# simon-donike/NIR-GAN

Measured on AMD Instinct MI355X. Metric: 256x256 RGB tiles/sec (G+D fwd+bwd+step), higher is better.
Workload: dtype f32 (3xbf16 split, 6 products, f32 accumulate) for the contractions with 32-channel runs incl. the Winograd plane GEMMs; exact f32 MFMA for the first / last layers; f32 everywhere else; 1 GPU; configs[1]: 6-block ResnetGenerator + 3-layer PatchGAN, bs=16/GPU, 256x256, GAN+L1, padding=0, fp32-equivalent MFMA (three bf16 terms, six products); global_batch=16, parallelism=dp1

## Files before the change

### include/nirgan_hip.h

```cpp
#ifndef NIRGAN_HIP_H
#define NIRGAN_HIP_H

#include <stdint.h>

#ifdef __cplusplus
extern "C" {
#endif

#define NIRGAN_MAX_TAPS 16

#define NIRGAN_OK 0
#define NIRGAN_ERR_ARG (-1)
#define NIRGAN_ERR_LAUNCH (-2)

#define NIRGAN_ACT_NONE 0
#define NIRGAN_ACT_RELU 1
#define NIRGAN_ACT_LRELU 2
#define NIRGAN_ACT_TANH 3

#define NIRGAN_BORDER_KEEP 0
#define NIRGAN_BORDER_REFLECT 1

int nirgan_version(void);
const char* nirgan_last_error(void);
// ... 142 lines not shown
    float* dbias;
} nirgan_tap_scatter_desc;
int nirgan_tap_scatter(const nirgan_tap_scatter_desc* d, void* stream);

typedef struct {
    const float* x; int x_hp, x_wp;
    int B, OH, OW, crop, C, k;
    const float* w;
    const float* bias; int act;
    float* out;
    const float* dout;
    float* dz; int64_t dz_elems;
    float* gx;
    float* gw; float* gbias;
    float* ws; int64_t ws_elems;
} nirgan_endconv_desc;
int64_t nirgan_endconv_dz_elems(int B, int OH, int OW);
int64_t nirgan_endconv_ws_elems(int B, int OH, int OW);
int nirgan_endconv_fwd(const nirgan_endconv_desc* d, void* stream);
int nirgan_endconv_dz(const nirgan_endconv_desc* d, void* stream);
int nirgan_endconv_dgrad(const nirgan_endconv_desc* d, void* stream);
int nirgan_endconv_wgrad(const nirgan_endconv_desc* d, void* stream);

int nirgan_lsgan(const float* pred, int64_t n, float target, float weight,
                 float* loss_out, float* grad, void* stream);

#define NIRGAN_GAN_VANILLA 1
#define NIRGAN_GAN_WGANGP 2
int nirgan_gan_loss(const float* pred, int64_t n, int mode, float target, float weight,
                    float* loss_out, float* grad, void* stream);

typedef struct {
    const float* rgb;
    const float* nir; const float* pred;
    int B, H, W;
    float w_l1, w_ndvi, w_ndwi, w_gndvi, w_savi, w_msavi, w_evi;
    int criterion;
    int log_all;
    const float* extra; int extra_cs, extra_c; float extra_scale;
    float* sums;
    float* grad_pred;
    float* ws; int64_t ws_elems;
} nirgan_pix_loss_desc;
#define NIRGAN_PIX_LOSS_WS_ELEMS 8192
int nirgan_pix_loss(const nirgan_pix_loss_desc* d, void* stream);

// ... 314 lines not shown
```

### nir-gan_amd/csrc/instnorm.hip

```cpp
#include "instnorm_dev.h"
#include <type_traits>

namespace {

__device__ __forceinline__ void rg_reduce2(f32x4& s1, f32x4& s2, f32x4* lds, int tid, int q4, int nrg) {
    lds[tid] = s1;
    lds[256 + tid] = s2;
    __syncthreads();
    if (tid < q4) {
        f32x4 a = lds[tid], b = lds[256 + tid];
        for (int r = 1; r < nrg; ++r) {
            a += lds[r * q4 + tid];
            b += lds[256 + r * q4 + tid];
        }
        s1 = a;
        s2 = b;
    }
    __syncthreads();
}

struct InFwd {
    const float* y; int y16; int HW, W, H, C;
    int norm; float eps;
    float* mean; float* rstd;
// ... 120 lines not shown
    int h = (start + rg) / p.W, w = (start + rg) - h * p.W;
    for (int pix = start + rg; pix < end; pix += nrg, w += nrg) {
        while (w >= p.W) { w -= p.W; ++h; }
        f32x4 v = (ldy4(yb, size_t(pix) * p.C + q * 4, p.y16) - mean) * rstd;
        v = act4(v, p.act, p.slope);
        if (rb) v += ld4(rb + size_t(h) * p.r_row + size_t(w) * p.C + q * 4);
        if (p.border == NIRGAN_BORDER_REFLECT && p.o_pad > 0) {
            int hs[3], wsx[3];
            const int nh = halo_images(h, p.H, p.o_pad, hs), nw = halo_images(w, p.W, p.o_pad, wsx);
            for (int i = 0; i < nh; ++i)
                for (int j = 0; j < nw; ++j) {
                    const size_t off = size_t(hs[i]) * p.o_row + size_t(wsx[j]) * p.C + q * 4;
                    if (ob) st4(ob + off, v);
                    st4_twin(ob16, off, v);
                }
        } else {
            const size_t off = size_t(h + p.o_pad) * p.o_row + size_t(w + p.o_pad) * p.C + q * 4;
            if (ob) st4(ob + off, v);
            st4_twin(ob16, off, v);
        }
    }
}

__global__ __launch_bounds__(256) void in_bwd_pass1_kernel(const InBwd p) {
    __shared__ f32x4 lds[512];
    const int tid = threadIdx.x, chunk = blockIdx.x, b = blockIdx.y;
    const int q4 = p.C / 4, nrg = in_nrg(p.C);
    const int q = tid % q4, rg = tid / q4;
    f32x4 s1 = {0, 0, 0, 0}, s2 = {0, 0, 0, 0};
    if (rg < nrg) {
        f32x4 mean = {0, 0, 0, 0}, rstd = {1, 1, 1, 1};
        if (p.norm) {
            mean = ld4(p.mean + size_t(b) * p.C + q * 4);
            rstd = ld4(p.rstd + size_t(b) * p.C + q * 4);
        }
        const float* gb = p.g ? y_at(p.g, size_t(b) * p.g_img, p.g16) : nullptr;
        const float* g2b = p.g2 ? p.g2 + size_t(b) * p.HW * p.C : nullptr;
        const float* yb = p.y ? y_at(p.y, size_t(b) * p.HW * p.C, p.y16) : nullptr;
        float* db = p.dy + size_t(b) * p.d_img + p.d_org;
        const int start = chunk * p.ppc;
        int end = start + p.ppc;
        end = end < p.HW ? end : p.HW;
        int h = (start + rg) / p.W, w = (start + rg) - h * p.W;
        for (int pix = start + rg; pix < end; pix += nrg, w += nrg) {
            while (w >= p.W) { w -= p.W; ++h; }
            const f32x4 ga = in_bwd_gsum(p, gb, g2b, h, w, pix, q);
            if (p.gsum_out) st4(p.gsum_out + (size_t(b) * p.HW + pix) * p.C + q * 4, ga);
            f32x4 z = {0, 0, 0, 0};
            const bool masked = p.act == NIRGAN_ACT_RELU || p.act == NIRGAN_ACT_LRELU;
            if (p.norm || masked) z = (ldy4(yb, size_t(pix) * p.C + q * 4, p.y16) - mean) * rstd;
            f32x4 gz = ga;
            if (masked) {
                const float neg = p.act == NIRGAN_ACT_RELU ? 0.f : p.slope;
#pragma unroll
                for (int i = 0; i < 4; ++i) gz[i] = z[i] > 0.f ? gz[i] : gz[i] * neg;
            }
            if (!p.norm) {
                const size_t off = size_t(h) * p.d_row + size_t(w) * p.C + q * 4;
                st4(db + off, gz);
                st4_twin(p.dy16 ? p.dy16 + size_t(b) * p.d_img + p.d_org : nullptr, off, gz);
            }
            s1 += gz;
            if (p.norm) s2 += gz * z;
        }
    }
    rg_reduce2(s1, s2, lds, tid, q4, nrg);
    if (tid < q4) {
        if (p.norm) {
            float* w = p.ws + (size_t(b) * p.nchunk + chunk) * 2 * p.C;
            st4(w + tid * 4, s1);
            st4(w + p.C + tid * 4, s2);
        } else if (p.dbias) {
            st4(p.ws + (size_t(b) * p.nchunk + chunk) * p.C + tid * 4, s1);
// ... 310 lines not shown
#define NG_APPLY_R(Y16, OUT, REFLECT) do { if (d->residual) NG_APPLY(Y16, OUT, REFLECT, true); else NG_APPLY(Y16, OUT, REFLECT, false); } while (0)
#define NG_APPLY_B(Y16, OUT) do { if (reflect) NG_APPLY_R(Y16, OUT, true); else NG_APPLY_R(Y16, OUT, false); } while (0)
#define NG_APPLY_O(Y16) do { if (out == 0) NG_APPLY_B(Y16, 0); else if (out == 1) NG_APPLY_B(Y16, 1); else NG_APPLY_B(Y16, 2); } while (0)
            if (p.y16) NG_APPLY_O(true); else NG_APPLY_O(false);
#undef NG_APPLY_O
#undef NG_APPLY_B
#undef NG_APPLY_R
#undef NG_APPLY
        } else {
            hipLaunchKernelGGL(in_apply_kernel, grid, dim3(256), 0, st, p);
        }
    }
    return nirgan_check_launch("instnorm_fwd");
}

extern "C" int nirgan_instnorm_bwd(const nirgan_in_bwd_desc* d, void* stream) {
    NG_REQUIRE(d && (d->dy || d->norm) && (d->g || d->g2), "instnorm_bwd: null pointer");
    const bool sums_only = d->dy == nullptr && d->dy_bf16 == nullptr;
    NG_REQUIRE(d->B > 0 && d->H > 0 && d->W > 0 && d->C >= 4 && d->C % 4 == 0 && d->C <= 1024, "instnorm_bwd: bad shape");
    NG_REQUIRE(!d->g || (d->g_hp == d->H + 2 * d->g_pad && d->g_wp == d->W + 2 * d->g_pad), "instnorm_bwd: g geometry mismatch");
    NG_REQUIRE(!d->g_fold || (d->g_pad < d->H && d->g_pad < d->W), "instnorm_bwd: fold halo wider than the image");
    NG_REQUIRE(sums_only || (d->d_hp == d->H + 2 * d->d_pad && d->d_wp == d->W + 2 * d->d_pad), "instnorm_bwd: dy geometry mismatch");
    const bool masked = d->act == NIRGAN_ACT_RELU || d->act == NIRGAN_ACT_LRELU;
    NG_REQUIRE(!(masked || d->norm) || d->y, "instnorm_bwd: y (pre-activation input of the block) required for the mask / statistics");
    NG_REQUIRE(!d->norm || (d->mean && d->rstd && d->ws), "instnorm_bwd: mean/rstd/ws required when norm");
    InBwd p = in_bwd_params(d);
    NG_REQUIRE(!d->dy_bf16 || (d->C % 8 == 0 && (reinterpret_cast<uintptr_t>(d->dy_bf16) & 15) == 0), "instnorm_bwd: bf16 twin needs C %% 8 == 0 and 16-byte alignment");
    NG_REQUIRE(!d->norm || d->ws_elems >= int64_t(d->B) * p.pchunks * 2 * d->C + int64_t(d->B) * 2 * d->C, "instnorm_bwd: ws too small");
    const bool pre = d->norm && d->sums_chunks > 0;
    NG_REQUIRE(!pre || d->gsum_out != nullptr || (d->g != nullptr && !d->g_fold && d->g2 == nullptr), "instnorm_bwd: sums_chunks needs the folded gradient in gsum_out, or a plain g (no fold, no g2)");
    hipStream_t st = static_cast<hipStream_t>(stream);
    NG_REQUIRE(d->norm || !d->dbias || (d->ws && d->ws_elems >= int64_t(d->B) * p.nchunk * d->C),
               "instnorm_bwd: dbias needs ws (one row of channel sums per block, summed in fixed order)");
    const long long gbig = (long long)p.g_img > (long long)p.d_img ? p.g_img : p.d_img;
    const bool fast = d->norm && d->g != nullptr && in_fast_ok(d->H, d->W, d->C, d->g_fold ? d->g_pad : 0, gbig > (long long)p.HW * p.C ? gbig : (long long)p.HW * p.C);
    const dim3 bgrid(p.nchunk, d->B);
#define NG_P1(Y16, G16, FOLD) hipLaunchKernelGGL((in_bwd_pass1_fast_kernel<Y16, G16, FOLD>), bgrid, dim3(256), 0, st, p)
#define NG_P1_F(Y16, G16) do { if (d->g_fold) NG_P1(Y16, G16, true); else NG_P1(Y16, G16, false); } while (0)
#define NG_P1_G(Y16) do { if (p.g16) NG_P1_F(Y16, true); else NG_P1_F(Y16, false); } while (0)
    if (!pre) {
        if (fast) { if (p.y16) NG_P1_G(true); else NG_P1_G(false); }
        else hipLaunchKernelGGL(in_bwd_pass1_kernel, bgrid, dim3(256), 0, st, p);
    }
#undef NG_P1_G
#undef NG_P1_F
#undef NG_P1
    if (!d->norm && d->dbias) return nirgan_colsum(d->ws, int64_t(d->B) * p.nchunk, d->C, d->dbias, 1, stream);
    if (d->norm) {
        hipLaunchKernelGGL(in_bwd_finalize_kernel, dim3(d->B, (d->C >= 64 && d->C % 64 == 0) ? d->C / 64 : 1), dim3(256), 0, st, p, d->B);
        if (!sums_only) {
            const bool fast2 = (d->g != nullptr ? fast : (d->gsum_out != nullptr && in_fast_ok(d->H, d->W, d->C, 0, (long long)p.d_img > (long long)p.HW * p.C ? p.d_img : (long long)p.HW * p.C)));
            const int dyo = d->dy && d->dy_bf16 ? 1 : (d->dy ? 0 : 2);
            const int B_ = d->B;
#define NG_P2(Y16, G16, FOLD, DY) hipLaunchKernelGGL((in_bwd_pass2_fast_kernel<Y16, G16, FOLD, DY>), bgrid, dim3(256), 0, st, p, B_)
#define NG_P2_D(Y16, G16, FOLD) do { if (dyo == 0) NG_P2(Y16, G16, FOLD, 0); else if (dyo == 1) NG_P2(Y16, G16, FOLD, 1); else NG_P2(Y16, G16, FOLD, 2); } while (0)
#define NG_P2_F(Y16, G16) do { if (d->g_fold && d->g) NG_P2_D(Y16, G16, true); else NG_P2_D(Y16, G16, false); } while (0)
#define NG_P2_G(Y16) do { if (p.g16) NG_P2_F(Y16, true); else NG_P2_F(Y16, false); } while (0)
            if (fast2) { if (p.y16) NG_P2_G(true); else NG_P2_G(false); }
            else hipLaunchKernelGGL(in_bwd_pass2_kernel, bgrid, dim3(256), 0, st, p, d->B);
#undef NG_P2_G
#undef NG_P2_F
#undef NG_P2_D
#undef NG_P2
        }
    }
// ... 3 lines not shown
```

### nir-gan_amd/nirgan_hip/engine.py

```python
from __future__ import annotations

import ctypes as C
from typing import Dict, List, Optional

import numpy as np
import torch

from . import geometry as G
from . import lib as L
from .options import OPT

IN_EPS = 1e-5


def _ptr(t: Optional[torch.Tensor]) -> Optional[int]:
    return None if t is None else t.data_ptr()


PRECISIONS = {"fp32": 0, "bf16": 1, "bf16x3": 2}


def precision_code(precision) -> int:
    if precision in PRECISIONS.values():
        return int(precision)
# ... 733 lines not shown
            continue
        for w in h.writers:
            if isinstance(w, L.InFwdDesc):
                w.out = None
            else:
                w.dy = None
            n += 1
        h.fp32_dead = True
    return n


def emit_in_bwd(plan: Plan, ctx: Ctx, *, g: Optional[Halo], g_fold=False, g2: Optional[Halo] = None, a: Optional[Halo] = None,
                act=L.ACT_NONE, slope=0.2, y: Optional[Halo] = None, stats=None, norm=True, dy: Halo, gsum: Optional[Halo] = None,
                dbias: Optional[torch.Tensor] = None, ws=None, shape=None, sums_only: bool = False, pre_sums: int = 0):
    B, H, W, Cc = shape
    d = L.InBwdDesc()
    if g is not None:
        assert g.H == H and g.W == W and g.C == Cc
        d.g, d.g_hp, d.g_wp, d.g_pad, d.g_fold = g.ptr_any(), g.hp, g.wp, g.pad, (1 if g_fold else 0)
        d.g_bf16 = 1 if g.is16 else 0
    if g2 is not None:
        assert g2.pad == 0
        d.g2 = g2.ptr
    d.act, d.slope = act, slope
    d.norm = 1 if norm else 0
    if y is not None:
        d.y, d.y_bf16 = y.ptr_any(), (1 if y.is16 else 0)
    if norm:
        d.mean, d.rstd = stats[0].data_ptr(), stats[1].data_ptr()
    if norm or dbias is not None:
        d.ws, d.ws_elems = ws.data_ptr(), ws.numel()
    d.B, d.H, d.W, d.C = B, H, W, Cc
    assert not sums_only or norm
    d.dy, d.d_hp, d.d_wp, d.d_pad = (None if sums_only else dy.operand_ptr()), dy.hp, dy.wp, dy.pad
    if dy.t16 is not None and not sums_only:
        d.dy_bf16 = dy.t16.data_ptr()
        dy.writers.append(d)
    if gsum is not None:
        d.gsum_out = gsum.ptr
    if pre_sums:
        assert norm and (gsum is not None or (g is not None and not g_fold and g2 is None))
        d.sums_chunks = pre_sums
    if dbias is not None:
        d.dbias = dbias.data_ptr()
    ctx.keep.append(d)
    plan.add("nirgan_instnorm_bwd", C.byref(d))
# ... 35 lines not shown
        self.inp, self.weight, self.bias = inp, weight, bias
        self.k, self.s, self.p, self.cout = k, s, p, cout
        self.norm, self.act, self.residual = norm, act, residual
        self.cin = inp.C if kind != "rowpacked" else cin_real
        ctx = eng.ctx
        if kind == "convT":
            self.OH, self.OW = inp.H * 2, inp.W * 2
        else:
            self.OH, self.OW = G.conv_out(inp.H, k, s, p), G.conv_out(inp.W, k, s, p)
        assert inp.pad >= (p if kind != "convT" else 1), (name, inp.pad, p)
        B = inp.B
        phase_px = self.OH * self.OW // (4 if kind == "convT" else 1)
        y16 = (ctx.precision == 1 and norm and OPT.bf16_y and OPT.epilogue_stats and cout % 4 == 0 and phase_px % 128 == 0
               and self.OH * self.OW >= min(OPT.epilogue_min_pixels, OPT.epilogue_min_pixels_bf16) and one_pass_tiles(B * phase_px, cout))
        self.y = Halo(ctx, B, self.OH, self.OW, cout, 0, bf16=y16)
        self.out = Halo(ctx, B, self.OH, self.OW, cout, out_pad, twin=True)
        eng.twinned.append(self.out)
        self.out_border = out_border
        self.stats = (ctx.zeros(B, cout), ctx.zeros(B, cout)) if norm else None
        eng.scratch.want(B, self.OH, self.OW, cout)
        self.keep_z = keep_z
        self.producer, self.defer_apply = None, False
        self.wino6, self.wino_fwd, self.wino_fwd_keeps_V = False, None, False

    def fold_producer_apply(self, producer: "ConvIN"):
        producer.defer_apply, self.producer = True, producer

    def emit_fwd(self, plan: Plan, pack: Plan):
        eng, ctx, inp = self.eng, self.eng.ctx, self.inp
        if self.kind == "conv" and wino_applicable(ctx, inp, self.k, self.s, self.p, self.cout, self.OH, self.OW):
            pre = self._emit_fwd_wino6(plan, pack)
        elif self.kind in ("conv", "rowpacked"):
            pre = self._emit_fwd_direct(plan, pack)
        else:
            descs = self._phase_descs(pack, inp, self.y, G.convT_fwd_phases(inp.H, inp.W, self.k, self.p),
                                      lambda hw: G.convT_fwd_pack(inp.C, self.cout, self.k, hw), self.bias, run=inp.C, N=self.cout,
                                      in_off=inp.pad - 1, out_off=0)
            pre = self._conv_stats(descs)
            emit_conv_group(plan, ctx, descs)
        emit_in_fwd(plan, ctx, self.y, self.out, norm=self.norm, act=(L.ACT_NONE if self.keep_z else self.act),
                    residual=self.residual, border=self.out_border, stats=self.stats, ws=(pre[2] if pre is not None else eng.scratch.get()),
                    stats_only=self.defer_apply, pre_stats=(pre[:2] if pre is not None else None))

    def _emit_fwd_wino6(self, plan: Plan, pack: Plan):
        eng, ctx, inp, k = self.eng, self.eng.ctx, self.inp, self.k
        keep = bool(eng.keep_wino_V)
        prod = self.producer
        xn = (prod.y, prod.stats, prod.act) if prod is not None and prod.defer_apply else None
        self.wino6 = True
        pre = sws = None
        if self.norm and OPT.epilogue_stats:
            T = _w6_tiles(inp.B, self.OH, self.OW, wino6_variant(k))
# ... 43 lines not shown
        return descs

    def _conv_stats(self, descs):
        pre = attach_conv_stats(self.eng.ctx, descs, self.bias) if self.norm else None
        self._y_fallback(pre, descs)
        return pre

    def _y_fallback(self, pre, descs):
        if self.y.is16 and pre is None:
            self.y = Halo(self.eng.ctx, self.inp.B, self.OH, self.OW, self.cout, 0)
            for d in descs:
                d.out, d.out_bf16 = self.y.ptr, 0

    def alloc_bwd(self, need_dgrad: bool):
        ctx, k = self.eng.ctx, self.k
        if self.kind == "convT":
            zpad = 1
        elif self.s == 1:
            zpad = k - 1 if need_dgrad else 0
        else:
            zpad = 1 if need_dgrad else 0
        self.dy = Halo(ctx, self.inp.B, self.OH, self.OW, self.cout, zpad, twin=True)
        self.eng.twinned.append(self.dy)

    def emit_bwd(self, plan: Plan, pack: Plan, *, g: Optional[Halo], g_fold=False, g2: Optional[Halo] = None,
                 gsum: Optional[Halo] = None, gw: Optional[torch.Tensor], gb: Optional[torch.Tensor], dgrad_out: Optional[Halo],
                 mask: Optional[Halo] = None, act=None):
        eng, ctx, inp = self.eng, self.eng.ctx, self.inp
        k, s, p = self.k, self.s, self.p
        act = self.act if act is None else act
        dy = self.dy
        w6_bwd = (self.kind == "conv" and s == 1 and gw is not None and dgrad_out is not None and dgrad_out.pad == p and dy.pad == k - 1
                  and wino_dgrad_applicable(ctx, k, s, dgrad_out, self.cout, inp.C) and inp.C > 64
                  and inp.pad == 1 and p == 1 and self.cout % 128 == 0)
        fuse_dy = (w6_bwd and k == 3 and self.norm and dy.t16 is None and OPT.fuse_dy_norm and wino6_variant(3) == 6
                   and act in (L.ACT_NONE, L.ACT_RELU, L.ACT_LRELU))
        scratch = eng.scratch.get()
        pre_sums, ws, gsum = (self._first_pass_from_w6_output(g, g_fold, g2, gsum, act)
                              or self._first_pass_from_conv_epilogues(g, g_fold, g2, gsum, act) or (0, scratch, gsum))
        nd = emit_in_bwd(plan, ctx, g=g, g_fold=g_fold, g2=g2, act=act, y=self.y, stats=self.stats, norm=self.norm, dy=self.dy, gsum=gsum,
                         dbias=(None if self.norm else gb),
                         ws=ws, shape=(inp.B, self.OH, self.OW, self.cout), pre_sums=pre_sums, sums_only=fuse_dy)
        if w6_bwd:
            self._emit_w6_backward(plan, pack, gw, dgrad_out, nd if fuse_dy else None)
        elif self.kind == "conv" and s == 1 and gw is not None and dgrad_out is not None:
            self._emit_paired_s1(plan, pack, gw, dgrad_out)
        else:
            if gw is not None:
                self._emit_wgrad(plan, gw)
            if dgrad_out is not None:
                self._emit_dgrad(plan, pack, dgrad_out, frozen=gw is None)

    def _first_pass_from_w6_output(self, g, g_fold, g2, gsum, act):
        ctx, inp = self.eng.ctx, self.inp
        od = g.w6_out_desc if g is not None else None
        if not (od is not None and od.r == 6 and g_fold and self.norm and g.pad == 1 and self.dy.t16 is None and OPT.fuse_inbwd):
            return None
        mo, Hp, Wp = _w6_geo(od.r if od.r else 3)[0], od.H, od.W
        if not (Hp == self.OH + 2 and Wp == self.OW + 2 and od.K == self.cout and od.B == inp.B and min(Hp, Wp) >= 6
                and (Hp - 3) // mo == (Hp - 1) // mo and (Wp - 3) // mo == (Wp - 1) // mo):
            return None
        chunks = (-(-Hp // mo)) * (-(-Wp // mo))
        if gsum is None:
# ... 179 lines not shown
```

### nir-gan_amd/nirgan_hip/lib.py

```python
from __future__ import annotations

import ctypes as C
import os

_HERE = os.path.dirname(os.path.abspath(__file__))
LIB_PATH = os.path.join(os.path.dirname(_HERE), "lib", "libnirgan_hip.so")

MAX_TAPS = 16
ACT_NONE, ACT_RELU, ACT_LRELU, ACT_TANH = 0, 1, 2, 3
BORDER_KEEP, BORDER_REFLECT = 0, 1
OP_CONV, OP_WGRAD, OP_IN_FWD, OP_IN_BWD = 1, 2, 3, 4

fp = C.c_void_p
i32, i64, f32 = C.c_int, C.c_int64, C.c_float


class ConvDesc(C.Structure):
    _fields_ = [("inp", fp), ("in_elems", i64), ("in_hp", i32), ("in_wp", i32), ("in_cs", i32),
                ("run", i32), ("in_stride", i32), ("in_oh", i32), ("in_ow", i32), ("ntaps", i32),
                ("tap_dh", i32 * MAX_TAPS), ("tap_dw", i32 * MAX_TAPS),
                ("w", fp), ("w_elems", i64), ("bias", fp),
                ("out", fp), ("out_elems", i64), ("out_hp", i32), ("out_wp", i32), ("out_cs", i32),
                ("out_stride", i32), ("out_oh", i32), ("out_ow", i32),
                ("B", i32), ("OH", i32), ("OW", i32), ("N", i32), ("zero_page", fp),
# ... 184 lines not shown

class RasterLookupDesc(C.Structure):
    _fields_ = [("points", fp), ("n_points", i32), ("H", i32), ("W", i32), ("dtype", i32), ("raster", fp),
                ("x0", C.c_double), ("dx", C.c_double), ("y0", C.c_double), ("dy", C.c_double),
                ("has_nodata", i32), ("nodata", i32), ("value", fp)]


class WinoDyDesc(C.Structure):
    _fields_ = [("dy", fp), ("dy_hp", i32), ("dy_wp", i32), ("dy_pad", i32), ("B", i32), ("H", i32), ("W", i32), ("K", i32),
                ("Yt", fp), ("Yt_elems", i64), ("r", i32)]


class Wino6Desc(C.Structure):
    _fields_ = [("x", fp), ("x_hp", i32), ("x_wp", i32), ("B", i32), ("H", i32), ("W", i32), ("C", i32), ("K", i32),
                ("U", fp), ("bias", fp), ("V", fp), ("V_elems", i64), ("M", fp), ("M_elems", i64), ("y", fp), ("zero_page", fp), ("r", i32), ("stats_ws", fp), ("stats_ws_elems", i64),
                ("fuse_y", fp), ("fuse_mean", fp), ("fuse_rstd", fp), ("fuse_g2", fp), ("fuse_gz", fp), ("fuse_part", fp), ("fuse_part_elems", i64),
                ("fuse_act", i32), ("fuse_slope", f32), ("algo", i32), ("U3", fp)]


W6_ONE_TILE, W6_DIRECT_TILE, W6_X3_R4 = 1, 3, 5
W6_PATCH_PER_THREAD, W6_PATCH_PER_LANES = 16, 17
WGRAD_ONE_UNIT, WGRAD_TILE128 = 1, 2
CONV_TILE128, CONV_X3_R4 = 1, 4


class EndConvDesc(C.Structure):
    _fields_ = [("x", fp), ("x_hp", i32), ("x_wp", i32), ("B", i32), ("OH", i32), ("OW", i32), ("crop", i32), ("C", i32), ("k", i32),
                ("w", fp), ("bias", fp), ("act", i32), ("out", fp), ("dout", fp), ("dz", fp), ("dz_elems", i64), ("gx", fp),
                ("gw", fp), ("gbias", fp), ("ws", fp), ("ws_elems", i64)]


class PlanEntry(C.Structure):
    _fields_ = [("op", i32), ("desc", fp)]


PROTOTYPES = {
    "nirgan_version": (i32, []),
    "nirgan_last_error": (C.c_char_p, []),
    "nirgan_conv_igemm": (i32, [C.POINTER(ConvDesc), fp]),
    "nirgan_wgrad_igemm": (i32, [C.POINTER(WgradDesc), fp]),
    "nirgan_conv_igemm_group": (i32, [C.POINTER(C.POINTER(ConvDesc)), i32, fp]),
    "nirgan_conv_wgrad_pair": (i32, [C.POINTER(ConvDesc), C.POINTER(WgradDesc), fp]),
    "nirgan_conv_kernel_name": (C.c_char_p, [C.POINTER(ConvDesc)]),
    "nirgan_wgrad_kernel_name": (C.c_char_p, [C.POINTER(WgradDesc)]),
    "nirgan_conv_wgrad_pair_kernel_name": (C.c_char_p, [C.POINTER(ConvDesc), C.POINTER(WgradDesc)]),
    "nirgan_reduce_rows": (i32, [fp, i32, i32, i32, fp, fp, i64, i32, i32, fp]),
# ... 44 lines not shown
    "nirgan_tile_metrics": (i32, [C.POINTER(TileMetricsDesc), fp]),
    "nirgan_window_stats": (i32, [C.POINTER(WindowStatsDesc), fp]),
    "nirgan_val_panel_ws_bytes": (i64, [i32, i32, i32]),
    "nirgan_val_panel": (i32, [C.POINTER(ValPanelDesc), fp]),
    "nirgan_class_metrics_ws_elems": (i64, [i32, i32, i32, i32]),
    "nirgan_class_metrics": (i32, [C.POINTER(ClassMetricsDesc), fp]),
    "nirgan_ssim_loss_ws_elems": (i64, [i32, i32, i32, i32]),
    "nirgan_ssim_loss": (i32, [C.POINTER(SsimLossDesc), fp]),
    "nirgan_emd_loss_ws_bytes": (i64, [i32, i64, i32]),
    "nirgan_emd_loss": (i32, [C.POINTER(EmdLossDesc), fp]),
    "nirgan_instnorm_ws_elems": (i64, [i32, i32, i32, i32]),
    "nirgan_instnorm_fwd": (i32, [C.POINTER(InFwdDesc), fp]),
    "nirgan_instnorm_bwd": (i32, [C.POINTER(InBwdDesc), fp]),
    "nirgan_nchw_to_halo": (i32, [fp, i32, i32, i32, i32, fp, i32, i32, i32, i32, i32, fp]),
    "nirgan_conv_channel_dgrad": (i32, [C.POINTER(ChanDgradDesc), fp]),
    "nirgan_tap_gather": (i32, [C.POINTER(TapGatherDesc), fp]),
    "nirgan_tap_scatter": (i32, [C.POINTER(TapScatterDesc), fp]),
    "nirgan_endconv_dz_elems": (i64, [i32, i32, i32]),
    "nirgan_endconv_ws_elems": (i64, [i32, i32, i32]),
    "nirgan_endconv_fwd": (i32, [C.POINTER(EndConvDesc), fp]),
    "nirgan_endconv_dz": (i32, [C.POINTER(EndConvDesc), fp]),
    "nirgan_endconv_dgrad": (i32, [C.POINTER(EndConvDesc), fp]),
    "nirgan_endconv_wgrad": (i32, [C.POINTER(EndConvDesc), fp]),
    "nirgan_lsgan": (i32, [fp, i64, f32, f32, fp, fp, fp]),
    "nirgan_gan_loss": (i32, [fp, i64, i32, f32, f32, fp, fp, fp]),
    "nirgan_pix_loss": (i32, [C.POINTER(PixLossDesc), fp]),
    "nirgan_pixmlp_fwd": (i32, [C.POINTER(PixMlpDesc), fp]),
    "nirgan_pixmlp_train": (i32, [C.POINTER(PixMlpDesc), fp]),
    "nirgan_pixmlp_ws_elems": (i64, [i32, i32, i32, i32]),
    "nirgan_pixdisc_ws_elems": (i64, [i32, i32, i32, i32]),
    "nirgan_pixdisc_fwd": (i32, [C.POINTER(PixDiscDesc), fp]),
    "nirgan_pixdisc_bwd": (i32, [C.POINTER(PixDiscDesc), fp]),
    "nirgan_adam": (i32, [fp, fp, fp, fp, i64, f32, f32, f32, f32, i32, fp]),
    "nirgan_bilinear_fwd": (i32, [fp, i32, i32, i32, fp, i32, i32, fp]),
    "nirgan_bilinear_bwd": (i32, [fp, i32, i32, i32, fp, i32, i32, fp]),
    "nirgan_inject_fwd": (i32, [C.POINTER(InjectFwdDesc), fp]),
    "nirgan_inject_bwd": (i32, [C.POINTER(InjectBwdDesc), fp]),
    "nirgan_param_scale_fwd": (i32, [fp, fp, fp, i64, fp]),
    "nirgan_param_scale_bwd": (i32, [fp, fp, fp, fp, fp, fp, i64, i64, fp]),
    "nirgan_colsum": (i32, [fp, i64, i32, fp, i32, fp]),
    "nirgan_fill": (i32, [fp, i64, f32, fp]),
    "nirgan_axpy": (i32, [fp, fp, i64, f32, fp]),
    "nirgan_run_plan": (i32, [C.POINTER(PlanEntry), i32, fp]),
}


# ... 52 lines not shown
```

### nir-gan_amd/nirgan_hip/nets.py

```python
from __future__ import annotations

import ctypes as C
from typing import Dict, Optional

import torch

from . import geometry as G
from . import lib as L
from .options import OPT
from .engine import (ConvIN, Ctx, Halo, LayerHost, Plan, TapPlaneConv, drop_dead_fp32_stores, emit_conv, grad_halo,
                     emit_deferred_reduce_rows, emit_w6_deferred_finishes, emit_wgrad, wino_applicable)


def generator_layout(n_blocks: int) -> dict:
    up0 = 10 + n_blocks
    return {"first": 1, "down": [4, 7], "blocks": list(range(10, 10 + n_blocks)), "up": [up0, up0 + 3], "last": up0 + 7}


class _Engine(LayerHost):
    def __init__(self, device, precision="fp32", keep_wino_V: bool = False):
        super().__init__(Ctx(device, precision), keep_wino_V)
        self.pack_fwd, self.pack_bwd = Plan(self.ctx), Plan(self.ctx)
        self.fwd, self.bwd = Plan(self.ctx), Plan(self.ctx)
        self._packed_version = -1
# ... 312 lines not shown
        self.bwd_pred = Plan(ctx)
        for plan, mode in ((b, "train"), (self.bwd_frozen, "input"), (self.bwd_pred, "pred")):
            frozen = mode != "train"

            def GW(i, what="weight"):
                return None if frozen else gr[f"model.{i}.{what}"]
            if not frozen:
                for k in ("model.0.bias", "model.11.bias"):
                    plan.add("nirgan_fill", gr[k].data_ptr(), gr[k].numel(), 0.0)
                ctx.rr_deferred = [] if OPT.batch_reduce else None
            self.C5.emit_bwd(plan, pk, GW(11), GW(11, "bias"))
            self.C4.emit_bwd(plan, pk, g=self.C5.gin, g_fold=False, gw=GW(8), gb=GW(8, "bias"), dgrad_out=self.g3p)
            if not frozen:
                emit_deferred_reduce_rows(plan, ctx, last=False)
                self.bwd_tail = (len(plan.ops), "model.8.weight", "model.11.bias")
            self.C3.emit_bwd(plan, pk, g=self.g3p, g_fold=False, gw=GW(5), gb=GW(5, "bias"), dgrad_out=self.g2)
            self.C2.emit_bwd(plan, pk, g=self.g2, gw=GW(2), gb=GW(2, "bias"), dgrad_out=self.g1)
            if not frozen:
                emit_deferred_reduce_rows(plan, ctx, last=False)
                self.bwd_mid = (len(plan.ops), "model.0.weight", "model.0.bias")
            self.C1.emit_bwd(plan, pk, g=self.g1, gw=GW(0), gb=GW(0, "bias"), dgrad_out=self.gx4 if mode == "input" else None)
            if not frozen:
                emit_deferred_reduce_rows(plan, ctx)
            if mode == "pred":
                d = L.ChanDgradDesc()
                dy, w = self.C1.dy, self.params["model.0.weight"]
                d.dy, d.dy_hp, d.dy_wp, d.dy_pad, d.C = dy.ptr, dy.hp, dy.wp, dy.pad, dy.C
                d.w, d.cin, d.k, d.stride, d.pad, d.channel = w.data_ptr(), 4, 4, 2, 1, 3
                d.B, d.H, d.W, d.out = B, self.H, self.W, self.gpred.data_ptr()
                ctx.keep.append(d)
                plan.add("nirgan_conv_channel_dgrad", C.byref(d))


class PixelDiscriminatorEngine(_DiscriminatorFrontEnd):

    FLAT_ELEMS = 8772

    def __init__(self, params: Dict[str, torch.Tensor], grads: Optional[Dict[str, torch.Tensor]], B: int, H: int, W: int,
                 need_backward: bool = True, precision="fp32"):
        w1 = params["net.0.weight"]
        super().__init__(params, grads, B, H, W, w1.device, precision)
        ctx = self.ctx
        ndf, in_nc = w1.shape[0], w1.shape[1]
        if in_nc != 4 or ndf != 64:
            raise NotImplementedError("the pixel discriminator of the MI355X path is built for cat(rgb, nir) = 4 channels and ndf = 64")
        if H * W < 2:
            raise ValueError(f"Expected more than 1 spatial element when training, got input size {torch.Size([B, 2 * ndf, H, W])}")
# ... 33 lines not shown
```

### nir-gan_amd/nirgan_hip/options.py

```python
from __future__ import annotations

import os


class Options:
    w6_gemm_algo: int = 0
    wgrad_algo: int = 0
    w6_pair: bool = True
    winograd: str = "f6"
    epilogue_stats: bool = True
    fuse_inbwd: bool = True
    epilogue_min_pixels: int = 16384
    epilogue_min_pixels_bf16: int = 1024
    fuse_dy_norm: bool = True
    dp_buckets: bool = True
    bf16_y: bool = True
    bf16_g: bool = True
    bf16_store_min_tiles: int = 100
    bf16_twin_only: bool = True
    fold_apply: bool = True
    tile256: bool = True
    batch_reduce: bool = True
    wgrad_target: int = 512
    split3: bool = True
    split3_wino: bool = True
    pair_phases: bool = True
    pair_pixels: bool = True
    x3_r4: bool = True
    endconv_direct: bool = True

    def reset(self):
        for k, v in vars(Options).items():
            if not k.startswith("_") and not callable(v):
                setattr(self, k, v)


    def update_from(self, text: str):
        for item in filter(None, (t.strip() for t in text.split(","))):
            k, _, v = item.partition("=")
            if not hasattr(Options, k) or k.startswith("_"):
                raise ValueError(f"NIRGAN_OPTIONS: unknown option '{k}'")
            cur = getattr(Options, k)
            setattr(self, k, (v.lower() in ("1", "true", "yes", "on")) if isinstance(cur, bool) else type(cur)(v))


OPT = Options()
if os.environ.get("NIRGAN_OPTIONS"):
    OPT.update_from(os.environ["NIRGAN_OPTIONS"])
```

Before: 1100 tiles/s.

## Add direct MFMA kernels for the discriminator's first 4->64 stride-2 conv

Adds a dedicated forward kernel for the PatchGAN's first Conv2d(4,64,4,s2,p1)+LeakyReLU. It gathers input patches straight from the padded input and runs exact f32 MFMA with a fused bias and activation epilogue, replacing the generic rowpacked conv path. It also adds direct wgrad and pred-dgrad kernels that take the LeakyReLU mask from the stored activation rather than the pre-activation, plus an instance-norm backward variant that does the same. The backward path sits behind an option that is off by default, so only the fused forward runs with default settings. Because the pre-activation is not stored, the mask is taken from the activation, which requires a positive slope.

```diff
diff --git a/include/nirgan_hip.h b/include/nirgan_hip.h
--- a/include/nirgan_hip.h
+++ b/include/nirgan_hip.h
@@ -188,6 +188,23 @@
 int nirgan_endconv_dgrad(const nirgan_endconv_desc* d, void* stream);
 int nirgan_endconv_wgrad(const nirgan_endconv_desc* d, void* stream);
 
+typedef struct {
+    const float* x;
+    int B, H, W, cin, cout, k;
+    const float* w;
+    const float* bias;
+    float slope;
+    float* a;
+    const float* g;
+    float* gw; float* gb;
+    float* ws; int64_t ws_elems;
+    float* gpred;
+} nirgan_firstconv_desc;
+int64_t nirgan_firstconv_ws_elems(int B, int H, int W);
+int nirgan_firstconv_fwd(const nirgan_firstconv_desc* d, void* stream);
+int nirgan_firstconv_wgrad(const nirgan_firstconv_desc* d, void* stream);
+int nirgan_firstconv_pred_dgrad(const nirgan_firstconv_desc* d, void* stream);
+
 int nirgan_lsgan(const float* pred, int64_t n, float target, float weight,
                  float* loss_out, float* grad, void* stream);
 
diff --git a/nir-gan_amd/csrc/firstconv.hip b/nir-gan_amd/csrc/firstconv.hip
--- /dev/null
+++ b/nir-gan_amd/csrc/firstconv.hip
@@ -0,0 +1,316 @@
+#include "common.h"
+
+namespace {
+
+constexpr int FC = 64;
+constexpr int FWD_MAX_BLOCKS = 512;
+constexpr int WG_MAX_BLOCKS = 512;
+constexpr int WG_ROW = FC * FC + FC;
+constexpr int PT_R = 14, PT_C = 30;
+
+struct FcP {
+    const float* x; int x_wp; int64_t x_img;
+    float* a; int a_wp; int64_t a_img;
+    const float* w; const float* bias; float slope;
+    int B, H, W, OH, OW;
+    const float* g;
+    float* ws; float* gw; float* gb; float* gpred;
+};
+
+__device__ __forceinline__ int uni(int v) { return __builtin_amdgcn_readfirstlane(v); }
+
+__global__ __launch_bounds__(256) void firstconv_fwd_kernel(const FcP p, const float* __restrict__ x, const float* __restrict__ w, float* __restrict__ a) {
+    const int lane = threadIdx.x & 63, half = lane >> 5, col = lane & 31;
+    float wa[32][2];
+#pragma unroll
+    for (int s = 0; s < 32; ++s) {
+        const int k = (s & 3) * 16 + (s >> 3) * 4 + 2 * ((s >> 2) & 1) + half;
+        wa[s][0] = w[col * FC + k];
+        wa[s][1] = w[(col + 32) * FC + k];
+    }
+    f32x4 bv[2][4];
+#pragma unroll
+    for (int t = 0; t < 2; ++t)
+#pragma unroll
+        for (int q = 0; q < 4; ++q) {
+            const f32x4 z = {0.f, 0.f, 0.f, 0.f};
+            bv[t][q] = p.bias ? *reinterpret_cast<const f32x4*>(p.bias + 32 * t + 8 * q + 4 * half) : z;
+        }
+    const int plane = p.OH * p.OW, npix = p.B * plane;
+    const int ntiles = (npix + 31) / 32, nwaves = uni(gridDim.x * 4);
+    const float slope = p.slope;
+
+    auto gather = [&](int tile, f32x4 (&xv)[4][2], int64_t& ooff) {
+        tile = tile < ntiles ? tile : ntiles - 1;
+        int pix = tile * 32 + col;
+        const bool ok = pix < npix;
+        pix = ok ? pix : npix - 1;
+        const int b = pix / plane, rem = pix - b * plane, oh = rem / p.OW, ow = rem - oh * p.OW;
+        const float* xp = x + (int64_t(b) * p.x_img + (int64_t(2 * oh) * p.x_wp + 2 * ow + half) * 4);
+#pragma unroll
+        for (int r = 0; r < 4; ++r)
+#pragma unroll
+            for (int j = 0; j < 2; ++j) xv[r][j] = *reinterpret_cast<const f32x4*>(xp + (r * p.x_wp + 2 * j) * 4);
+        ooff = ok ? int64_t(b) * p.a_img + (int64_t(oh + 1) * p.a_wp + ow + 1) * FC : -1;
+    };
+    auto tile_out = [&](const f32x4 (&xv)[4][2], int64_t ooff) {
+        f32x16 acc0 = {0}, acc1 = {0};
+#pragma unroll
+        for (int s = 0; s < 32; ++s) {
+            const float b = xv[s >> 3][(s >> 2) & 1][s & 3];
+            acc0 = __builtin_amdgcn_mfma_f32_32x32x2f32(wa[s][0], b, acc0, 0, 0, 0);
+            acc1 = __builtin_amdgcn_mfma_f32_32x32x2f32(wa[s][1], b, acc1, 0, 0, 0);
+        }
+        if (ooff < 0) return;
+        float* o = a + ooff + 4 * half;
+#pragma unroll
+        for (int q = 0; q < 4; ++q) {
+            f32x4 v0, v1;
+#pragma unroll
+            for (int i = 0; i < 4; ++i) {
+                const float z0 = acc0[4 * q + i] + bv[0][q][i], z1 = acc1[4 * q + i] + bv[1][q][i];
+                v0[i] = z0 > 0.f ? z0 : z0 * slope;
+                v1[i] = z1 > 0.f ? z1 : z1 * slope;
+            }
+            *reinterpret_cast<f32x4*>(o + 8 * q) = v0;
+            *reinterpret_cast<f32x4*>(o + 32 + 8 * q) = v1;
+        }
+    };
+    int tile = uni(blockIdx.x * 4 + (threadIdx.x >> 6));
+    f32x4 x0[4][2], x1[4][2];
+    int64_t o0, o1;
+    gather(tile, x0, o0);
+    while (true) {
+        if (tile >= ntiles) break;
+        gather(tile + nwaves, x1, o1);
+        asm volatile("" ::: "memory");
+        tile_out(x0, o0);
+        tile += nwaves;
+        if (tile >= ntiles) break;
+        gather(tile + nwaves, x0, o0);
+        asm volatile("" ::: "memory");
+        tile_out(x1, o1);
+        tile += nwaves;
+    }
+}
+
+__global__ __launch_bounds__(256) void firstconv_wgrad_kernel(const FcP p, const float* __restrict__ g, const float* __restrict__ a,
+                                                              const float* __restrict__ x, float* __restrict__ ws) {
+    __shared__ float red[WG_ROW];
+    const int lane = threadIdx.x & 63, wv = threadIdx.x >> 6, half = lane >> 5, col = lane & 31;
+    const int upr = (p.OW + 15) / 16, nunits = p.B * p.OH * upr, nwaves = uni(gridDim.x * 4);
+    const int xlane = ((col >> 3) * p.x_wp + ((col >> 1) & 3)) * 4 + 2 * (col & 1);
+    const float slope = p.slope;
+    struct Buf { f32x2 g[8], a[8], x[8]; };
+    auto load = [&](int unit, Buf& f) {
+        unit = unit < nunits ? unit : nunits - 1;
+        const int row = unit / upr, ow0 = (unit - row * upr) * 16;
+        const int b = row / p.OH, oh = row - b * p.OH;
+        const float* gu = g + int64_t(row) * p.OW * FC + 2 * col;
+        const float* au = a + (int64_t(b) * p.a_img + (int64_t(oh + 1) * p.a_wp + 1) * FC) + 2 * col;
+        const float* xu = x + (int64_t(b) * p.x_img + int64_t(2 * oh) * p.x_wp * 4) + xlane;
+#pragma unroll
+        for (int j = 0; j < 8; ++j) {
+            int ow = ow0 + 2 * j + half;
+            ow = ow < p.OW ? ow : p.OW - 1;
+            f.g[j] = *reinterpret_cast<const f32x2*>(gu + ow * FC);
+            f.a[j] = *reinterpret_cast<const f32x2*>(au + ow * FC);
+            f.x[j] = *reinterpret_cast<const f32x2*>(xu + ow * 8);
+        }
+    };
+    f32x16 acc[2][2] = {{{0}, {0}}, {{0}, {0}}};
+    float sb0 = 0.f, sb1 = 0.f;
+    auto mma = [&](int unit, const Buf& f) {
+        const int ow0 = (unit % upr) * 16;
+#pragma unroll
+        for (int j = 0; j < 8; ++j) {
+            const bool ok = ow0 + 2 * j + half < p.OW;
+            const float d0 = ok ? f.g[j][0] * (f.a[j][0] > 0.f ? 1.f : slope) : 0.f;
+            const float d1 = ok ? f.g[j][1] * (f.a[j][1] > 0.f ? 1.f : slope) : 0.f;
+            sb0 += d0;
+            sb1 += d1;
+            acc[0][0] = __builtin_amdgcn_mfma_f32_32x32x2f32(d0, f.x[j][0], acc[0][0], 0, 0, 0);
+            acc[0][1] = __builtin_amdgcn_mfma_f32_32x32x2f32(d0, f.x[j][1], acc[0][1], 0, 0, 0);
+            acc[1][0] = __builtin_amdgcn_mfma_f32_32x32x2f32(d1, f.x[j][0], acc[1][0], 0, 0, 0);
+            acc[1][1] = __builtin_amdgcn_mfma_f32_32x32x2f32(d1, f.x[j][1], acc[1][1], 0, 0, 0);
+        }
+    };
+    Buf f0, f1;
+    int unit = uni(blockIdx.x * 4 + wv);
+    load(unit, f0);
+    while (true) {
+        if (unit >= nunits) break;
+        load(unit + nwaves, f1);
+        asm volatile("" ::: "memory");
+        mma(unit, f0);
+        unit += nwaves;
+        if (unit >= nunits) break;
+        load(unit + nwaves, f0);
+        asm volatile("" ::: "memory");
+        mma(unit, f1);
+        unit += nwaves;
+    }
+    sb0 += __shfl_xor(sb0, 32, 64);
+    sb1 += __shfl_xor(sb1, 32, 64);
+    for (int w4 = 0; w4 < 4; ++w4) {
+        if (wv == w4) {
+#pragma unroll
+            for (int mt = 0; mt < 2; ++mt)
+#pragma unroll
+                for (int r = 0; r < 16; ++r) {
+                    const int n = 2 * ((r & 3) + 8 * (r >> 2) + 4 * half) + mt;
+#pragma unroll
+                    for (int nt = 0; nt < 2; ++nt) {
+                        const int i = n * FC + 2 * col + nt;
+                        red[i] = w4 == 0 ? acc[mt][nt][r] : red[i] + acc[mt][nt][r];
+                    }
+                }
+            if (half == 0) {
+                const int i = FC * FC + 2 * col;
+                red[i] = w4 == 0 ? sb0 : red[i] + sb0;
+                red[i + 1] = w4 == 0 ? sb1 : red[i + 1] + sb1;
+            }
+        }
+        __syncthreads();
+    }
+    float* o = ws + int64_t(blockIdx.x) * WG_ROW;
+    for (int i = threadIdx.x; i < WG_ROW; i += 256) o[i] = red[i];
+}
+
+__global__ __launch_bounds__(256) void firstconv_wgrad_finish_kernel(const float* __restrict__ ws, int nblk, float* __restrict__ gw, float* __restrict__ gb) {
+    __shared__ float part[16][17];
+    const int o = threadIdx.x & 15, sl = threadIdx.x >> 4;
+    const int i = blockIdx.x * 16 + o;
+    float s = 0.f;
+#pragma unroll 8
+    for (int k = sl; k < nblk; k += 16) s += ws[int64_t(k) * WG_ROW + i];
+    part[sl][o] = s;
+    __syncthreads();
+    if (threadIdx.x < 16) {
+        float t = 0.f;
+#pragma unroll
+        for (int k = 0; k < 16; ++k) t += part[k][threadIdx.x];
+        const int j = blockIdx.x * 16 + threadIdx.x;
+        if (j < FC * FC) {
+            const int n = j >> 6, k = j & 63;
+            gw[n * FC + (k & 3) * 16 + (k >> 2)] = t;
+        } else if (gb != nullptr) {
+            gb[j - FC * FC] += t;
+        }
+    }
+}
+
+__global__ __launch_bounds__(256) void firstconv_pred_dgrad_kernel(const FcP p, const float* __restrict__ g, const float* __restrict__ a,
+                                                                   const float* __restrict__ w, float* __restrict__ out) {
+    __shared__ float T[(PT_R + 2) * (PT_C + 2) * 16];
+    const int tid = threadIdx.x, lane = tid & 63, wv = tid >> 6, m = lane & 15, kq = lane >> 4;
+    const int tc = (p.OW + PT_C - 1) / PT_C, tr = (p.OH + PT_R - 1) / PT_R;
+    const int tile = blockIdx.x;
+    const int b = tile / (tr * tc), r0 = (tile / tc) % tr * PT_R, c0 = tile % tc * PT_C;
+    float wb[16];
+#pragma unroll
+    for (int s = 0; s < 16; ++s) wb[s] = w[(16 * kq + s) * FC + 48 + m];
+    const float slope = p.slope;
+    const float* gb_ = g + int64_t(b) * p.OH * p.OW * FC + 16 * kq;
+    const float* ab_ = a + int64_t(b) * p.a_img + 16 * kq;
+    constexpr int GROUPS = (PT_R + 2) * (PT_C + 2) / 16;
+#pragma unroll 2
+    for (int it = 0; it < GROUPS / 4; ++it) {
+        const int grp = it * 4 + wv, px = grp * 16 + m;
+        const int oh = r0 - 1 + px / (PT_C + 2), ow = c0 - 1 + px % (PT_C + 2);
+        const bool ok = oh >= 0 && oh < p.OH && ow >= 0 && ow < p.OW;
+        const int ohc = ok ? oh : 0, owc = ok ? ow : 0;
+        const float* gp = gb_ + (int64_t(ohc) * p.OW + owc) * FC;
+        const float* ap = ab_ + (int64_t(ohc + 1) * p.a_wp + owc + 1) * FC;
+        f32x4 gv[4], av[4];
+#pragma unroll
+        for (int i = 0; i < 4; ++i) {
+            gv[i] = *reinterpret_cast<const f32x4*>(gp + 4 * i);
+            av[i] = *reinterpret_cast<const f32x4*>(ap + 4 * i);
+        }
+        f32x4 acc = {0.f, 0.f, 0.f, 0.f};
+#pragma unroll
+        for (int s = 0; s < 16; ++s) {
+            const float dz = ok ? gv[s >> 2][s & 3] * (av[s >> 2][s & 3] > 0.f ? 1.f : slope) : 0.f;
+            acc = __builtin_amdgcn_mfma_f32_16x16x4f32(dz, wb[s], acc, 0, 0, 0);
+        }
+#pragma unroll
+        for (int r = 0; r < 4; ++r) T[(grp * 16 + 4 * kq + r) * 16 + m] = acc[r];
+    }
+    __syncthreads();
+    for (int i = tid; i < 4 * PT_R * PT_C; i += 256) {
+        const int hl = i / (2 * PT_C), wl = i - hl * (2 * PT_C);
+        const int h = 2 * r0 + hl, ww = 2 * c0 + wl;
+        if (h >= p.H || ww >= p.W) continue;
+        const int kh = (hl + 1) & 1, lr = (hl + 1 - kh) / 2 + 1;
+        const int kw = (wl + 1) & 1, lc = (wl + 1 - kw) / 2 + 1;
+        const float* t0 = T + (lr * (PT_C + 2) + lc) * 16 + kh * 4 + kw;
+        const float* t1 = t0 - (PT_C + 2) * 16 + 8;
+        out[(int64_t(b) * p.H + h) * p.W + ww] = (t0[0] + t0[-16 + 2]) + (t1[0] + t1[-16 + 2]);
+    }
+}
+
+int wgrad_blocks(int B, int OH, int OW) {
+    const int64_t b = (int64_t(B) * OH * ((OW + 15) / 16) + 3) / 4;
+    return int(b < WG_MAX_BLOCKS ? b : WG_MAX_BLOCKS);
+}
+
+int fill_params(const nirgan_firstconv_desc* d, FcP& p, const char* what) {
+    NG_REQUIRE(d != nullptr, "%s: null descriptor", what);
+    NG_REQUIRE(d->cout == FC && d->cin == 4 && d->k == 4, "%s: the direct kernels cover Conv2d(4, 64, 4, stride 2, padding 1) only (cin=%d cout=%d k=%d)", what, d->cin, d->cout, d->k);
+    NG_REQUIRE(d->B > 0 && d->H > 0 && d->W > 0 && d->H % 2 == 0 && d->W % 2 == 0, "%s: bad shape (H and W must be even)", what);
+    NG_REQUIRE(d->slope > 0.f, "%s: the mask is taken from the activation: the slope must be positive", what);
+    p.B = d->B; p.H = d->H; p.W = d->W; p.OH = d->H / 2; p.OW = d->W / 2;
+    NG_REQUIRE(int64_t(d->B) * (p.OH + 2) * (p.OW + 2) * FC < (1ll << 31) && int64_t(d->B) * (d->H + 2) * (d->W + 2) * 4 < (1ll << 31), "%s: problem too large", what);
+    p.x = d->x; p.x_wp = d->W + 2; p.x_img = int64_t(d->H + 2) * (d->W + 2) * 4;
+    p.a = d->a; p.a_wp = p.OW + 2; p.a_img = int64_t(p.OH + 2) * (p.OW + 2) * FC;
+    p.w = d->w; p.bias = d->bias; p.slope = d->slope;
+    p.g = d->g; p.ws = d->ws; p.gw = d->gw; p.gb = d->gb; p.gpred = d->gpred;
+    return NIRGAN_OK;
+}
+
+}
+
+extern "C" int64_t nirgan_firstconv_ws_elems(int B, int H, int W) {
+    if (B <= 0 || H <= 0 || W <= 0 || H % 2 || W % 2) return 0;
+    return int64_t(wgrad_blocks(B, H / 2, W / 2)) * WG_ROW;
+}
+
+extern "C" int nirgan_firstconv_fwd(const nirgan_firstconv_desc* d, void* stream) {
+    FcP p;
+    const int rc = fill_params(d, p, "firstconv_fwd");
+    if (rc != NIRGAN_OK) return rc;
+    NG_REQUIRE(d->x && d->w && d->a, "firstconv_fwd: null pointer");
+    NG_REQUIRE(ng_aligned16(d->x) && ng_aligned16(d->a) && ng_aligned16(d->w) && ng_aligned16(d->bias), "firstconv_fwd: x, w, bias and a must be 16-byte aligned");
+    const int64_t blocks = ((int64_t(p.B) * p.OH * p.OW + 31) / 32 + 3) / 4;
+    hipLaunchKernelGGL(firstconv_fwd_kernel, dim3(int(blocks < FWD_MAX_BLOCKS ? blocks : FWD_MAX_BLOCKS)), dim3(256), 0, static_cast<hipStream_t>(stream),
+                       p, p.x, p.w, p.a);
+    return nirgan_check_launch("firstconv_fwd");
+}
+
+extern "C" int nirgan_firstconv_wgrad(const nirgan_firstconv_desc* d, void* stream) {
+    FcP p;
+    const int rc = fill_params(d, p, "firstconv_wgrad");
+    if (rc != NIRGAN_OK) return rc;
+    NG_REQUIRE(d->x && d->a && d->g && d->gw && d->ws, "firstconv_wgrad: null pointer");
+    NG_REQUIRE(ng_aligned16(d->x) && ng_aligned16(d->a) && ng_aligned16(d->g) && ng_aligned16(d->ws), "firstconv_wgrad: x, a, g and ws must be 16-byte aligned");
+    NG_REQUIRE(d->ws_elems >= nirgan_firstconv_ws_elems(d->B, d->H, d->W), "firstconv_wgrad: partials workspace too small (nirgan_firstconv_ws_elems)");
+    const int nblk = wgrad_blocks(p.B, p.OH, p.OW);
+    hipStream_t st = static_cast<hipStream_t>(stream);
+    hipLaunchKernelGGL(firstconv_wgrad_kernel, dim3(nblk), dim3(256), 0, st, p, p.g, (const float*)p.a, p.x, p.ws);
+    hipLaunchKernelGGL(firstconv_wgrad_finish_kernel, dim3(WG_ROW / 16), dim3(256), 0, st, (const float*)p.ws, nblk, p.gw, p.gb);
+    return nirgan_check_launch("firstconv_wgrad");
+}
+
+extern "C" int nirgan_firstconv_pred_dgrad(const nirgan_firstconv_desc* d, void* stream) {
+    FcP p;
+    const int rc = fill_params(d, p, "firstconv_pred_dgrad");
+    if (rc != NIRGAN_OK) return rc;
+    NG_REQUIRE(d->a && d->g && d->w && d->gpred, "firstconv_pred_dgrad: null pointer");
+    NG_REQUIRE(ng_aligned16(d->a) && ng_aligned16(d->g) && ng_aligned16(d->w), "firstconv_pred_dgrad: a, g and w must be 16-byte aligned");
+    const int64_t blocks = int64_t(p.B) * ((p.OH + PT_R - 1) / PT_R) * ((p.OW + PT_C - 1) / PT_C);
+    NG_REQUIRE(blocks < (1ll << 31), "firstconv_pred_dgrad: problem too large");
+    hipLaunchKernelGGL(firstconv_pred_dgrad_kernel, dim3(int(blocks)), dim3(256), 0, static_cast<hipStream_t>(stream),
+                       p, p.g, (const float*)p.a, p.w, p.gpred);
+    return nirgan_check_launch("firstconv_pred_dgrad");
+}
diff --git a/nir-gan_amd/csrc/instnorm.hip b/nir-gan_amd/csrc/instnorm.hip
--- a/nir-gan_amd/csrc/instnorm.hip
+++ b/nir-gan_amd/csrc/instnorm.hip
@@ -166,6 +166,7 @@
     }
 }
 
+template <bool AMASK>
 __global__ __launch_bounds__(256) void in_bwd_pass1_kernel(const InBwd p) {
     __shared__ f32x4 lds[512];
     const int tid = threadIdx.x, chunk = blockIdx.x, b = blockIdx.y;
@@ -181,6 +182,7 @@
         const float* gb = p.g ? y_at(p.g, size_t(b) * p.g_img, p.g16) : nullptr;
         const float* g2b = p.g2 ? p.g2 + size_t(b) * p.HW * p.C : nullptr;
         const float* yb = p.y ? y_at(p.y, size_t(b) * p.HW * p.C, p.y16) : nullptr;
+        const float* ab = AMASK ? p.a + size_t(b) * p.a_img + p.a_org : nullptr;
         float* db = p.dy + size_t(b) * p.d_img + p.d_org;
         const int start = chunk * p.ppc;
         int end = start + p.ppc;
@@ -192,7 +194,8 @@
             if (p.gsum_out) st4(p.gsum_out + (size_t(b) * p.HW + pix) * p.C + q * 4, ga);
             f32x4 z = {0, 0, 0, 0};
             const bool masked = p.act == NIRGAN_ACT_RELU || p.act == NIRGAN_ACT_LRELU;
-            if (p.norm || masked) z = (ldy4(yb, size_t(pix) * p.C + q * 4, p.y16) - mean) * rstd;
+            if constexpr (AMASK) z = ld4(ab + size_t(h) * p.a_row + size_t(w) * p.C + q * 4);
+            else if (p.norm || masked) z = (ldy4(yb, size_t(pix) * p.C + q * 4, p.y16) - mean) * rstd;
             f32x4 gz = ga;
             if (masked) {
                 const float neg = p.act == NIRGAN_ACT_RELU ? 0.f : p.slope;
@@ -549,7 +552,9 @@
     NG_REQUIRE(!d->g_fold || (d->g_pad < d->H && d->g_pad < d->W), "instnorm_bwd: fold halo wider than the image");
     NG_REQUIRE(sums_only || (d->d_hp == d->H + 2 * d->d_pad && d->d_wp == d->W + 2 * d->d_pad), "instnorm_bwd: dy geometry mismatch");
     const bool masked = d->act == NIRGAN_ACT_RELU || d->act == NIRGAN_ACT_LRELU;
-    NG_REQUIRE(!(masked || d->norm) || d->y, "instnorm_bwd: y (pre-activation input of the block) required for the mask / statistics");
+    const bool mask_from_a = !d->y && d->a && !d->norm && d->act == NIRGAN_ACT_LRELU && d->slope > 0.f &&
+                             d->a_hp == d->H + 2 * d->a_pad && d->a_wp == d->W + 2 * d->a_pad && d->a_pad >= 0 && ng_aligned16(d->a);
+    NG_REQUIRE(!(masked || d->norm) || d->y || mask_from_a, "instnorm_bwd: y (pre-activation input of the block) required for the mask / statistics");
     NG_REQUIRE(!d->norm || (d->mean && d->rstd && d->ws), "instnorm_bwd: mean/rstd/ws required when norm");
     InBwd p = in_bwd_params(d);
     NG_REQUIRE(!d->dy_bf16 || (d->C % 8 == 0 && (reinterpret_cast<uintptr_t>(d->dy_bf16) & 15) == 0), "instnorm_bwd: bf16 twin needs C %% 8 == 0 and 16-byte alignment");
@@ -567,7 +572,8 @@
 #define NG_P1_G(Y16) do { if (p.g16) NG_P1_F(Y16, true); else NG_P1_F(Y16, false); } while (0)
     if (!pre) {
         if (fast) { if (p.y16) NG_P1_G(true); else NG_P1_G(false); }
-        else hipLaunchKernelGGL(in_bwd_pass1_kernel, bgrid, dim3(256), 0, st, p);
+        else if (!d->y && mask_from_a) hipLaunchKernelGGL(in_bwd_pass1_kernel<true>, bgrid, dim3(256), 0, st, p);
+        else hipLaunchKernelGGL(in_bwd_pass1_kernel<false>, bgrid, dim3(256), 0, st, p);
     }
 #undef NG_P1_G
 #undef NG_P1_F
diff --git a/nir-gan_amd/nirgan_hip/engine.py b/nir-gan_amd/nirgan_hip/engine.py
--- a/nir-gan_amd/nirgan_hip/engine.py
+++ b/nir-gan_amd/nirgan_hip/engine.py
@@ -779,6 +779,9 @@
     if g2 is not None:
         assert g2.pad == 0
         d.g2 = g2.ptr
+    if a is not None and y is None:
+        assert not norm and act == L.ACT_LRELU and (a.H, a.W, a.C) == (H, W, Cc)
+        d.a, d.a_hp, d.a_wp, d.a_pad = a.ptr, a.hp, a.wp, a.pad
     d.act, d.slope = act, slope
     d.norm = 1 if norm else 0
     if y is not None:
@@ -860,12 +863,44 @@
         self.keep_z = keep_z
         self.producer, self.defer_apply = None, False
         self.wino6, self.wino_fwd, self.wino_fwd_keeps_V = False, None, False
+        self.firstconv = self._firstconv_applies(out_pad, residual)
+        self.firstconv_bwd = self.firstconv and OPT.firstconv_direct_bwd
+        self.fc_ws = None
+
+    def _firstconv_applies(self, out_pad, residual) -> bool:
+        inp, be = self.inp, L.backend()
+        return bool(OPT.firstconv_direct and self.kind == "rowpacked" and self.cout == 64 and self.cin == 4 and inp.C == 4
+                    and (self.k, self.s, self.p) == (4, 2, 1) and inp.pad == 1 and out_pad == 1 and self.out_border == L.BORDER_KEEP
+                    and not self.norm and self.act == L.ACT_LRELU and residual is None and not self.keep_z
+                    and inp.H % 2 == 0 and inp.W % 2 == 0 and self.out.t16 is None
+                    and self.weight.data_ptr() % 16 == 0 and (self.bias is None or self.bias.data_ptr() % 16 == 0)
+                    and all(hasattr(be, n) for n in ("nirgan_firstconv_fwd", "nirgan_firstconv_wgrad", "nirgan_firstconv_pred_dgrad",
+                                                     "nirgan_firstconv_ws_elems")))
+
+    def _firstconv_desc(self, g: Optional[Halo] = None):
+        inp = self.inp
+        d = L.FirstConvDesc()
+        d.x, d.B, d.H, d.W, d.cin, d.cout, d.k = inp.ptr, inp.B, inp.H, inp.W, self.cin, self.cout, self.k
+        d.w, d.bias, d.slope, d.a = self.weight.data_ptr(), _ptr(self.bias), 0.2, self.out.ptr
+        if g is not None:
+            assert g.pad == 0 and not g.is16 and (g.H, g.W, g.C) == (self.OH, self.OW, self.cout)
+            d.g = g.ptr
+        self.eng.ctx.keep.append(d)
+        return d
+
+    def emit_firstconv_pred_dgrad(self, plan: Plan, g: Halo, gpred: torch.Tensor):
+        d = self._firstconv_desc(g)
+        d.gpred = gpred.data_ptr()
+        plan.add("nirgan_firstconv_pred_dgrad", C.byref(d))
 
     def fold_producer_apply(self, producer: "ConvIN"):
         producer.defer_apply, self.producer = True, producer
 
     def emit_fwd(self, plan: Plan, pack: Plan):
         eng, ctx, inp = self.eng, self.eng.ctx, self.inp
+        if self.firstconv:
+            plan.add("nirgan_firstconv_fwd", C.byref(self._firstconv_desc()))
+            return
         if self.kind == "conv" and wino_applicable(ctx, inp, self.k, self.s, self.p, self.cout, self.OH, self.OW):
             pre = self._emit_fwd_wino6(plan, pack)
         elif self.kind in ("conv", "rowpacked"):
@@ -955,6 +990,8 @@
             zpad = 1 if need_dgrad else 0
         self.dy = Halo(ctx, self.inp.B, self.OH, self.OW, self.cout, zpad, twin=True)
         self.eng.twinned.append(self.dy)
+        if self.firstconv_bwd:
+            self.fc_ws = ctx.zeros(int(L.backend().nirgan_firstconv_ws_elems(self.inp.B, self.inp.H, self.inp.W)))
 
     def emit_bwd(self, plan: Plan, pack: Plan, *, g: Optional[Halo], g_fold=False, g2: Optional[Halo] = None,
                  gsum: Optional[Halo] = None, gw: Optional[torch.Tensor], gb: Optional[torch.Tensor], dgrad_out: Optional[Halo],
@@ -963,6 +1000,13 @@
         k, s, p = self.k, self.s, self.p
         act = self.act if act is None else act
         dy = self.dy
+        if self.firstconv_bwd and dgrad_out is None:
+            assert g is not None and not g_fold and g2 is None and gsum is None and mask is None and act == self.act
+            if gw is not None:
+                d = self._firstconv_desc(g)
+                d.gw, d.gb, d.ws, d.ws_elems = gw.data_ptr(), _ptr(gb), self.fc_ws.data_ptr(), self.fc_ws.numel()
+                plan.add("nirgan_firstconv_wgrad", C.byref(d))
+            return
         w6_bwd = (self.kind == "conv" and s == 1 and gw is not None and dgrad_out is not None and dgrad_out.pad == p and dy.pad == k - 1
                   and wino_dgrad_applicable(ctx, k, s, dgrad_out, self.cout, inp.C) and inp.C > 64
                   and inp.pad == 1 and p == 1 and self.cout % 128 == 0)
@@ -971,7 +1015,8 @@
         scratch = eng.scratch.get()
         pre_sums, ws, gsum = (self._first_pass_from_w6_output(g, g_fold, g2, gsum, act)
                               or self._first_pass_from_conv_epilogues(g, g_fold, g2, gsum, act) or (0, scratch, gsum))
-        nd = emit_in_bwd(plan, ctx, g=g, g_fold=g_fold, g2=g2, act=act, y=self.y, stats=self.stats, norm=self.norm, dy=self.dy, gsum=gsum,
+        nd = emit_in_bwd(plan, ctx, g=g, g_fold=g_fold, g2=g2, act=act, y=(None if self.firstconv else self.y),
+                         a=(self.out if self.firstconv else None), stats=self.stats, norm=self.norm, dy=self.dy, gsum=gsum,
                          dbias=(None if self.norm else gb),
                          ws=ws, shape=(inp.B, self.OH, self.OW, self.cout), pre_sums=pre_sums, sums_only=fuse_dy)
         if w6_bwd:
diff --git a/nir-gan_amd/nirgan_hip/lib.py b/nir-gan_amd/nirgan_hip/lib.py
--- a/nir-gan_amd/nirgan_hip/lib.py
+++ b/nir-gan_amd/nirgan_hip/lib.py
@@ -230,6 +230,11 @@
 W6_PATCH_PER_THREAD, W6_PATCH_PER_LANES = 16, 17
 WGRAD_ONE_UNIT, WGRAD_TILE128 = 1, 2
 CONV_TILE128, CONV_X3_R4 = 1, 4
+
+
+class FirstConvDesc(C.Structure):
+    _fields_ = [("x", fp), ("B", i32), ("H", i32), ("W", i32), ("cin", i32), ("cout", i32), ("k", i32), ("w", fp), ("bias", fp),
+                ("slope", f32), ("a", fp), ("g", fp), ("gw", fp), ("gb", fp), ("ws", fp), ("ws_elems", i64), ("gpred", fp)]
 
 
 class EndConvDesc(C.Structure):
@@ -320,6 +325,10 @@
     "nirgan_endconv_dz": (i32, [C.POINTER(EndConvDesc), fp]),
     "nirgan_endconv_dgrad": (i32, [C.POINTER(EndConvDesc), fp]),
     "nirgan_endconv_wgrad": (i32, [C.POINTER(EndConvDesc), fp]),
+    "nirgan_firstconv_ws_elems": (i64, [i32, i32, i32]),
+    "nirgan_firstconv_fwd": (i32, [C.POINTER(FirstConvDesc), fp]),
+    "nirgan_firstconv_wgrad": (i32, [C.POINTER(FirstConvDesc), fp]),
+    "nirgan_firstconv_pred_dgrad": (i32, [C.POINTER(FirstConvDesc), fp]),
     "nirgan_lsgan": (i32, [fp, i64, f32, f32, fp, fp, fp]),
     "nirgan_gan_loss": (i32, [fp, i64, i32, f32, f32, fp, fp, fp]),
     "nirgan_pix_loss": (i32, [C.POINTER(PixLossDesc), fp]),
diff --git a/nir-gan_amd/nirgan_hip/nets.py b/nir-gan_amd/nirgan_hip/nets.py
--- a/nir-gan_amd/nirgan_hip/nets.py
+++ b/nir-gan_amd/nirgan_hip/nets.py
@@ -358,7 +358,9 @@
             self.C1.emit_bwd(plan, pk, g=self.g1, gw=GW(0), gb=GW(0, "bias"), dgrad_out=self.gx4 if mode == "input" else None)
             if not frozen:
                 emit_deferred_reduce_rows(plan, ctx)
-            if mode == "pred":
+            if mode == "pred" and self.C1.firstconv_bwd:
+                self.C1.emit_firstconv_pred_dgrad(plan, self.g1, self.gpred)
+            elif mode == "pred":
                 d = L.ChanDgradDesc()
                 dy, w = self.C1.dy, self.params["model.0.weight"]
                 d.dy, d.dy_hp, d.dy_wp, d.dy_pad, d.C = dy.ptr, dy.hp, dy.wp, dy.pad, dy.C
diff --git a/nir-gan_amd/nirgan_hip/options.py b/nir-gan_amd/nirgan_hip/options.py
--- a/nir-gan_amd/nirgan_hip/options.py
+++ b/nir-gan_amd/nirgan_hip/options.py
@@ -28,6 +28,8 @@
     pair_pixels: bool = True
     x3_r4: bool = True
     endconv_direct: bool = True
+    firstconv_direct: bool = True
+    firstconv_direct_bwd: bool = False
 
     def reset(self):
         for k, v in vars(Options).items():
```

After: 1108 tiles/s, median of 6. No clear change (+0.7%).
